# LLNL/ExaConstit

Measured on AMD Instinct MI355X. Metric: quadrature-point constitutive updates/s + Newton-PCG iter/s, 128^3 hex RVE, higher is better.
Workload: dtype f64

## Files before the change

### exaconstit_amd/csrc/capi.hip

```cpp
#include <climits>
#include "exa_internal.hpp"
#include <cstring>
#include <cstdio>

int exa_launch_model_setup(exa_ctx*, double, double*, const double*, const double*, const double*, const double*, double*, double*, double*, hipStream_t);
int exa_launch_model_setup_rec(exa_ctx*, double, double*, const double*, const double*, const double*, const double*, double*, double*, hipStream_t);
int exa_launch_model_setup_p2(exa_ctx*, double, double*, const double*, const double*, const double*, const double*, double*, double*, double*, bool, hipStream_t);
int exa_launch_model_setup_aos_rec(exa_ctx*, double, double*, const double*, const double*, const double*, const double*, double*, double*, hipStream_t);
int exa_launch_init_state(exa_ctx*, double*, const double*, const double*, hipStream_t);
int exa_launch_state_normalize(exa_ctx*, double*, hipStream_t);
int exa_launch_nfev_hist(exa_ctx*, const double*, int*, hipStream_t);
int exa_launch_selftest_km_math(const double*, double*, int, hipStream_t);
int exa_launch_calc_dp(exa_ctx*, const double*, double*, hipStream_t);
int exa_launch_jacobians(exa_ctx*, const double*, double*, hipStream_t);
int exa_launch_jacobians_from_geom(exa_ctx*, const double*, double*, hipStream_t);
int exa_launch_grad_calc(exa_ctx*, const double*, const double*, double*, hipStream_t);
int exa_launch_residual_setup(exa_ctx*, const double*, const double*, hipStream_t);
int exa_launch_residual_apply(exa_ctx*, double*, hipStream_t);
int exa_launch_residual_p1(exa_ctx*, const double*, const double*, double*, bool, hipStream_t);
int exa_launch_grad_setup_pa(exa_ctx*, double, const double*, const double*, hipStream_t);
int exa_launch_grad_apply_p1(exa_ctx*, const double*, double*, bool, const uint8_t*, const double*, hipStream_t, bool trans = false, int blk0 = 0, int nblk_range = -1);
int exa_launch_grad_diag_p1(exa_ctx*, double*, hipStream_t);
int exa_launch_assemble_ea_p1(exa_ctx*, hipStream_t);
int exa_launch_ea_apply_p1(exa_ctx*, const double*, double*, bool, const uint8_t*, const double*, hipStream_t);
int exa_launch_ea_diag_p1(exa_ctx*, double*, hipStream_t);
int exa_launch_ea_export_p1(exa_ctx*, double*, hipStream_t);
int exa_launch_restrict(exa_ctx*, const double*, double*, hipStream_t);
// ... 37 lines not shown
      if (!told) { told = true; std::fprintf(stderr, "exaconstit_hip: Kocks-Mecking kinetics with p = %g, q = %g: the regime p, q != 1 is not pinned to a reference vector (DESIGN.md section 5)\n", ctx->mp.p, ctx->mp.q); }
   }
   exa_build_ref_elem(ctx->p, ctx->G_host, ctx->W_host);
   bool ok = true;
   ok = ok && hipMalloc(&ctx->G_dev, sizeof(double) * ctx->G_host.size()) == hipSuccess;
   ok = ok && hipMalloc(&ctx->W_dev, sizeof(double) * ctx->W_host.size()) == hipSuccess;
   ok = ok && hipMalloc(&ctx->fail_count_dev, sizeof(int)) == hipSuccess;
   ctx->scratch_bytes = sizeof(double) * VOL_AVG_BLOCKS * 64;
   ok = ok && hipMalloc(&ctx->scratch_dev, ctx->scratch_bytes) == hipSuccess;
   if (ok) {
      ok = ok && hipMemcpy(ctx->G_dev, ctx->G_host.data(), sizeof(double) * ctx->G_host.size(), hipMemcpyHostToDevice) == hipSuccess;
      ok = ok && hipMemcpy(ctx->W_dev, ctx->W_host.data(), sizeof(double) * ctx->W_host.size(), hipMemcpyHostToDevice) == hipSuccess;
      ok = ok && hipMemset(ctx->fail_count_dev, 0, sizeof(int)) == hipSuccess;
   }
   if (!ok) { std::fprintf(stderr, "exa_create: device allocation failed\n"); exa_destroy(ctx); set(EXA_ERR_HIP); return nullptr; }
   set(EXA_OK);
   return ctx;
}

void exa_destroy(exa_ctx* ctx) {
   if (!ctx) return;
   (void)hipFree(ctx->n2e_off); (void)hipFree(ctx->n2e_idx); (void)hipFree(ctx->ev_det);
   (void)hipFree(ctx->G_dev); (void)hipFree(ctx->W_dev); (void)hipFree(ctx->fail_count_dev); (void)hipFree(ctx->tail_dev); (void)hipFree(ctx->tail2_dev); (void)hipFree(ctx->resume_dev[0]); (void)hipFree(ctx->resume_dev[1]); (void)hipFree(ctx->scratch_dev);
   (void)hipFree(ctx->dmat); (void)hipFree(ctx->pa); (void)hipFree(ctx->emat); (void)hipFree(ctx->eDS); (void)hipFree(ctx->T1_dev); (void)hipFree(ctx->pa_c); (void)hipFree(ctx->tbuf); (void)hipFree(ctx->vgrad_ref);
   delete ctx;
}

const char* exa_last_error(const exa_ctx* ctx) { return ctx ? ctx->err.c_str() : "null context"; }
int exa_num_state_vars(const exa_ctx* ctx) { return ctx ? ctx->nstatev : EXA_ERR_ARG; }
int exa_nodes_per_elem(const exa_ctx* ctx) { return ctx ? ctx->n : EXA_ERR_ARG; }
int exa_qpts_per_elem(const exa_ctx* ctx) { return ctx ? ctx->Q : EXA_ERR_ARG; }

int exa_shape_table(const exa_ctx* ctx, double* G_host, double* W_host) {
   if (!ctx) return EXA_ERR_ARG;
   if (G_host) std::memcpy(G_host, ctx->G_host.data(), sizeof(double) * ctx->G_host.size());
   if (W_host) std::memcpy(W_host, ctx->W_host.data(), sizeof(double) * ctx->W_host.size());
   return EXA_OK;
}

int exa_set_quadrature_layout(exa_ctx* ctx, int layout) {
   if (!ctx || (layout != EXA_QLAYOUT_AOS && layout != EXA_QLAYOUT_EB64)) return fail(ctx, EXA_ERR_ARG, "exa_set_quadrature_layout: bad argument");
   if (layout == EXA_QLAYOUT_EB64 && !((ctx->p == 1 && ctx->cfg.integ == EXA_INTEG_FULL) || ctx->p == 2))
      return fail(ctx, EXA_ERR_UNSUPPORTED, "exa_set_quadrature_layout: the element-blocked layout is built for p = 1 full integration and for p = 2");
   ctx->qblk = (layout == EXA_QLAYOUT_EB64); ctx->have_resid = false; ctx->have_grad = false;
   return EXA_OK;
}
// ... 16 lines not shown

extern "C" int exa_choose_newton_cap(const int* hist64, double tail_cost);
static int cap_controller(exa_ctx* ctx, int rc, const double* state1, exa_stream s) {
   if (rc != EXA_OK || !ctx->cap_auto) return rc;
   ctx->cap_calls++;
   if (!(ctx->cap_calls <= 4 || ctx->cap_calls % 4 == 0)) return rc;
   int h[64];
   if (int r = exa_model_nfev_hist(ctx, state1, h, s)) return r;
   return exa_set_newton_caps(ctx, exa_choose_newton_cap(h, ctx->cap_tail_cost), 0, ctx->tail_resume);
}

int exa_set_newton_cap_auto(exa_ctx* ctx, int mode, double tail_cost) {
   if (!ctx || mode < 0 || mode > 2) return fail(ctx, EXA_ERR_ARG, "exa_set_newton_cap_auto: mode 0 (off), 1 (Kocks-Mecking models only) or 2 (every model)");
   if (mode && ctx->P >= (int64_t)INT32_MAX) return fail(ctx, EXA_ERR_ARG, "exa_set_newton_cap_auto: the deferred-point list holds 32-bit point ids (P < 2^31)");
   const bool km = ecmdev::kin_is_km(ctx->mp.kin);
   ctx->cap_auto = (mode == 2 || (mode == 1 && km)) ? 1 : 0;
   ctx->cap_tail_cost = tail_cost > 0.0 ? tail_cost : (km ? 1.5 : 4.0);
   ctx->cap_calls = 0;
   if (!mode) { ctx->newton_cap = 0; ctx->newton_cap2 = 0; }
   return EXA_OK;
}
int exa_get_newton_cap(exa_ctx* ctx) { return ctx ? ctx->newton_cap : EXA_ERR_ARG; }

int exa_model_setup(exa_ctx* ctx, double dt, const double* J, const double* vel, const double* stress0, const double* state0,
                    double* stress1, double* state1, double* ddsdde, exa_stream s) {
   if (!ctx || !J || !vel || !stress0 || !state0 || !stress1 || !state1 || !ddsdde) return fail(ctx, EXA_ERR_ARG, "exa_model_setup: null pointer");
   if (!(dt > 0.0)) return fail(ctx, EXA_ERR_ARG, "exa_model_setup: dt must be positive");
   return cap_controller(ctx, exa_launch_model_setup(ctx, dt, const_cast<double*>(J), vel, nullptr, stress0, state0, stress1, state1, ddsdde, S(s)), state1, s);
}

int exa_model_setup_lvec(exa_ctx* ctx, double dt, const double* x_lvec, const double* v_lvec, const double* stress0, const double* state0,
                         double* stress1, double* state1, double* ddsdde, double* J_out, exa_stream s) {
   if (!ctx || !x_lvec || !v_lvec || !stress0 || !state0 || !stress1 || !state1 || !ddsdde || !J_out) return fail(ctx, EXA_ERR_ARG, "exa_model_setup_lvec: null pointer");
   if (!ctx->conn) return fail(ctx, EXA_ERR_STATE, "exa_model_setup_lvec: call exa_set_connectivity first");
   if (!(dt > 0.0)) return fail(ctx, EXA_ERR_ARG, "exa_model_setup_lvec: dt must be positive");
   return cap_controller(ctx, exa_launch_model_setup(ctx, dt, J_out, v_lvec, x_lvec, stress0, state0, stress1, state1, ddsdde, S(s)), state1, s);
}

int exa_model_setup_lvec_records(exa_ctx* ctx, double dt, const double* x_lvec, const double* v_lvec, const double* stress0, const double* state0,
                                 double* stress1, double* state1, double* J_out, exa_stream s) {
   if (!ctx || !x_lvec || !v_lvec || !stress0 || !state0 || !stress1 || !state1) return fail(ctx, EXA_ERR_ARG, "exa_model_setup_lvec_records: null pointer");
   if (!ctx->conn) return fail(ctx, EXA_ERR_STATE, "exa_model_setup_lvec_records: call exa_set_connectivity first");
   if (!(dt > 0.0)) return fail(ctx, EXA_ERR_ARG, "exa_model_setup_lvec_records: dt must be positive");
   const bool p1 = ctx->p == 1 && ctx->cfg.integ == EXA_INTEG_FULL, p2 = ctx->p == 2;
   if (!(p1 || p2) || (!ctx->qblk && !p1) || ctx->tangent_form != EXA_TANGENT_DEV5_BULK || !(ctx->cfg.assembly == EXA_ASSEMBLY_PA || ctx->ea_matfree))
      return fail(ctx, EXA_ERR_UNSUPPORTED, "exa_model_setup_lvec_records: needs p = 1 full integration (either layout) or p = 2 (element-blocked layout), the compact tangent form and PA or matrix-free EA");
   if (p2 && !J_out) return fail(ctx, EXA_ERR_ARG, "exa_model_setup_lvec_records: at p = 2 the Jacobian field is not optional (the pre-pass writes it, the launch and the residual read it)");
   const int npair = p1 ? PAC_PAIRS : PAC_PAIRS_GEO;
   if (ctx->pa_c && ctx->pac_pairs != npair) return fail(ctx, EXA_ERR_STATE, "exa_model_setup_lvec_records: compact records of another shape exist");
   if (!ctx->pa_c) {
      ctx->pac_pairs = npair;
      EXA_HIP_CHECK(ctx, hipMalloc(&ctx->pa_c, (size_t)((ctx->E + PA_BLK - 1) / PA_BLK) * ctx->Q * 2 * npair * PA_BLK * sizeof(double)));
      EXA_HIP_CHECK(ctx, hipMemsetAsync(ctx->pa_c, 0, (size_t)((ctx->E + PA_BLK - 1) / PA_BLK) * ctx->Q * 2 * npair * PA_BLK * sizeof(double), S(s)));
   }
   const int rc = p2 ? exa_launch_model_setup_p2(ctx, dt, J_out, v_lvec, x_lvec, stress0, state0, stress1, state1, nullptr, true, S(s))
                     : !ctx->qblk ? exa_launch_model_setup_aos_rec(ctx, dt, J_out, v_lvec, x_lvec, stress0, state0, stress1, state1, S(s))
                     : exa_launch_model_setup_rec(ctx, dt, J_out, v_lvec, x_lvec, stress0, state0, stress1, state1, S(s));
   if (rc == EXA_OK) { ctx->have_grad = true; ctx->emat_valid = false; ctx->grad_records_only = true; }
   return cap_controller(ctx, rc, state1, s);
}

const int* exa_model_fail_counter_dev(exa_ctx* ctx) { return ctx ? ctx->fail_count_dev : nullptr; }

int exa_model_status(exa_ctx* ctx, exa_stream s) {
   if (!ctx) return EXA_ERR_ARG;
   int h = 0;
// ... 27 lines not shown
   EXA_HIP_CHECK(ctx, hipStreamSynchronize(S(s)));
   return EXA_OK;
}
int exa_selftest_km_math(const double* x_dev, double* out_dev, int n, exa_stream s) {
   if (!x_dev || !out_dev || n <= 0) return EXA_ERR_ARG;
   return exa_launch_selftest_km_math(x_dev, out_dev, n, S(s));
}
int exa_model_tail_count(exa_ctx* ctx, exa_stream s) {
   if (!ctx) return EXA_ERR_ARG;
   if (!ctx->tail_dev || ctx->newton_cap <= 0) return 0;
   int h = 0;
   EXA_HIP_CHECK(ctx, hipMemcpyAsync(&h, ctx->tail_dev, sizeof(int), hipMemcpyDeviceToHost, S(s)));
   EXA_HIP_CHECK(ctx, hipStreamSynchronize(S(s)));
   return h;
}

int exa_calc_dp(exa_ctx* ctx, const double* state, double* dp, exa_stream s) {
   if (!ctx || !state || !dp) return fail(ctx, EXA_ERR_ARG, "exa_calc_dp: null pointer");
   return exa_launch_calc_dp(ctx, state, dp, S(s));
}

int exa_jacobians(exa_ctx* ctx, const double* xe, double* J, exa_stream s) {
   if (!ctx || !xe || !J) return fail(ctx, EXA_ERR_ARG, "exa_jacobians: null pointer");
   return exa_launch_jacobians(ctx, xe, J, S(s));
}

int exa_jacobians_from_geom(exa_ctx* ctx, const double* gj, double* J, exa_stream s) {
   if (!ctx || !gj || !J) return fail(ctx, EXA_ERR_ARG, "exa_jacobians_from_geom: null pointer");
   return exa_launch_jacobians_from_geom(ctx, gj, J, S(s));
}

int exa_grad_calc(exa_ctx* ctx, const double* J, const double* fe, double* out, exa_stream s) {
   if (!ctx || !J || !fe || !out) return fail(ctx, EXA_ERR_ARG, "exa_grad_calc: null pointer");
   return exa_launch_grad_calc(ctx, J, fe, out, S(s));
}

int exa_residual_setup(exa_ctx* ctx, const double* J, const double* stress1, exa_stream s) {
   if (!ctx || !J || !stress1) return fail(ctx, EXA_ERR_ARG, "exa_residual_setup: null pointer");
   if (ctx->qblk) return fail(ctx, EXA_ERR_UNSUPPORTED, "exa_residual_setup: E-vector residual is AOS-only; with the element-blocked layout use exa_residual_lvec");
   ctx->have_resid = true;
   if (ctx->cfg.integ == EXA_INTEG_BBAR) {
      if (!ctx->eDS) EXA_HIP_CHECK(ctx, hipMalloc(&ctx->eDS, sizeof(double) * 3 * ctx->n * PA_BLK * (size_t)((ctx->E + PA_BLK - 1) / PA_BLK)));
      ctx->resid_J = J; ctx->resid_S = stress1;
      return exa_launch_eds(ctx, J, S(s));
   }
   if (!ctx->dmat) EXA_HIP_CHECK(ctx, hipMalloc(&ctx->dmat, sizeof(double) * 9 * ctx->P));
   return exa_launch_residual_setup(ctx, J, stress1, S(s));
}

int exa_residual_apply(exa_ctx* ctx, double* y, exa_stream s) {
   if (!ctx || !y) return fail(ctx, EXA_ERR_ARG, "exa_residual_apply: null pointer");
// ... 43 lines not shown

int exa_set_ea_matrix_free(exa_ctx* ctx, int on) {
   if (!ctx) return EXA_ERR_ARG;
   ctx->ea_matfree = on != 0; return EXA_OK;
}

int exa_grad_setup(exa_ctx* ctx, double dt, const double* J, const double* C, exa_stream s) {
   if (!ctx || !J || !C) return fail(ctx, EXA_ERR_ARG, "exa_grad_setup: null pointer");
   if (!ctx->pa) { EXA_HIP_CHECK(ctx, hipMalloc(&ctx->pa, pa_bytes(ctx->E, ctx->Q))); EXA_HIP_CHECK(ctx, hipMemsetAsync(ctx->pa, 0, pa_bytes(ctx->E, ctx->Q), S(s))); }
   if (ctx->tangent_form == EXA_TANGENT_DEV5_BULK_GEO && !ctx->pa_c) {
      ctx->pac_pairs = PAC_PAIRS_GEO;
      EXA_HIP_CHECK(ctx, hipMalloc(&ctx->pa_c, (size_t)((ctx->E + PA_BLK - 1) / PA_BLK) * ctx->Q * 2 * ctx->pac_pairs * PA_BLK * sizeof(double)));
   }
   if (ctx->tangent_form == EXA_TANGENT_DEV5_BULK && !ctx->pa_c) {
      const bool p1 = ctx->p == 1 && ctx->cfg.integ == EXA_INTEG_FULL && (ctx->cfg.assembly == EXA_ASSEMBLY_PA || ctx->ea_matfree);
      const bool p2 = ctx->n == 27 && (ctx->cfg.assembly == EXA_ASSEMBLY_PA || ctx->ea_matfree);
      if (p1 || p2) {
         ctx->pac_pairs = p1 ? PAC_PAIRS : PAC_PAIRS_GEO;
         EXA_HIP_CHECK(ctx, hipMalloc(&ctx->pa_c, (size_t)((ctx->E + PA_BLK - 1) / PA_BLK) * ctx->Q * 2 * ctx->pac_pairs * PA_BLK * sizeof(double)));
      }
   }
   int rc = exa_launch_grad_setup_pa(ctx, dt, J, C, S(s));
   if (rc) return rc;
   ctx->grad_records_only = false;
   if (ctx->cfg.assembly == EXA_ASSEMBLY_EA) {
      const bool bbar = ctx->cfg.integ == EXA_INTEG_BBAR;
      ctx->ea_generic = bbar || ctx->p != 1;
      if (bbar) {
         if (!ctx->eDS) EXA_HIP_CHECK(ctx, hipMalloc(&ctx->eDS, sizeof(double) * 3 * ctx->n * PA_BLK * (size_t)((ctx->E + PA_BLK - 1) / PA_BLK)));
         rc = exa_launch_eds(ctx, J, S(s));
         if (rc) return rc;
      }
      ctx->emat_valid = false;
      if (!ea_from_records(ctx)) rc = assemble_ea(ctx, S(s));
   } else if (ctx->p != 1) {
      if (!ctx->tbuf) EXA_HIP_CHECK(ctx, hipMalloc(&ctx->tbuf, sizeof(double) * 9 * ctx->P));
   }
   ctx->have_grad = (rc == EXA_OK);
   return rc;
}

int exa_grad_apply(exa_ctx* ctx, const double* x, double* y, exa_stream s) {
   if (!ctx || !x || !y) return fail(ctx, EXA_ERR_ARG, "exa_grad_apply: null pointer");
   if (!ctx->have_grad) return fail(ctx, EXA_ERR_STATE, "exa_grad_apply called before exa_grad_setup");
   if (ctx->grad_records_only) return fail(ctx, EXA_ERR_STATE, "exa_grad_apply: the gradient data are the compact records of exa_model_setup_lvec_records; call exa_grad_setup for the full records");
   if (ctx->cfg.assembly == EXA_ASSEMBLY_EA) {
// ... 136 lines not shown
```

### exaconstit_amd/csrc/exa_internal.hpp

```cpp
#pragma once
#include <hip/hip_runtime.h>
#include <string>
#include <vector>
#include <cstdint>
#include <cstdlib>
#include "../../include/exaconstit_hip.h"
#include "ecm_device.hpp"

#define EXA_HIP_CHECK(ctx, call)                                                                 \
   do {                                                                                          \
      hipError_t e_ = (call);                                                                    \
      if (e_ != hipSuccess) { (ctx)->err = std::string(#call) + ": " + hipGetErrorString(e_); return EXA_ERR_HIP; } \
   } while (0)

constexpr int PA_SLOTS = 46;
constexpr int PA_PAIRS = 23;
constexpr int PA_BLK = 64;

struct exa_ctx {
   exa_config cfg;
   ecmdev::MatParams mp;
   int p, n, Q, E;
   int64_t P;
   int nstatev;
   int device;
   std::string err;
   std::vector<double> G_host, W_host;
   double* G_dev = nullptr; double* W_dev = nullptr;
   double* dmat = nullptr;
   double* pa = nullptr;
   double* emat = nullptr;
   double* T1_dev = nullptr;
   double* eDS = nullptr;
   double* tbuf = nullptr;
   double* vgrad_ref = nullptr;
   const double* resid_J = nullptr; const double* resid_S = nullptr;
   bool ea_generic = false;
   bool ea_matfree = false, emat_valid = false;
   bool qblk = false;
   bool aos_stage = true;
   bool have_resid = false, have_grad = false;
   bool pa_lazy = false; const double* lazy_J = nullptr; const double* lazy_C = nullptr; double lazy_dt = 0.0;
   bool grad_records_only = false;
   const int32_t* conn = nullptr; int nnodes = 0;
   double* pa_c = nullptr;
   int tangent_form = 0;
   int pac_pairs = 0;
   int det = 0; int32_t* n2e_off = nullptr; int32_t* n2e_idx = nullptr; double* ev_det = nullptr; int det_nnodes = 0; const int32_t* det_conn = nullptr;
   const double* coords_lvec = nullptr;
   int* fail_count_dev = nullptr;
   int newton_cap = 0; int* tail_dev = nullptr;
   int newton_cap2 = 0; int* tail2_dev = nullptr;
   int tail_resume = 1; double* resume_dev[2] = { nullptr, nullptr };
   int cap_auto = 0; double cap_tail_cost = 0.0; long cap_calls = 0;
   double* scratch_dev = nullptr; size_t scratch_bytes = 0;
   double hist_init[ecmdev::NUM_HIST];
};

int exa_ensure_p2_tables(struct exa_ctx* ctx);
void exa_build_ref_elem(int p, std::vector<double>& G, std::vector<double>& W);
void exa_build_1d_tables(int p, std::vector<double>& T1, std::vector<int>& nat);
bool exa_fill_mat_params(const exa_config& cfg, ecmdev::MatParams& mp, double* hist_init, std::string& err);

struct QView { int64_t base; int stride; };
template <bool QB>
// ... 84 lines not shown
```

### exaconstit_amd/csrc/pa_kernels.hip

```cpp
#include "exa_internal.hpp"
#include <cstdlib>
#include <cstring>

namespace {

constexpr double GL0 = 0.21132486540518713, GL1 = 0.78867513459481287;
constexpr double gl_pt(int i) { return i == 0 ? GL0 : GL1; }
constexpr int VX[8] = { 0, 1, 1, 0, 0, 1, 1, 0 }, VY[8] = { 0, 0, 1, 1, 0, 0, 1, 1 }, VZ[8] = { 0, 0, 0, 0, 1, 1, 1, 1 };
constexpr double n1(int v, double x) { return v ? x : 1.0 - x; }
constexpr double d1(int v) { return v ? 1.0 : -1.0; }
constexpr double G1(int a, int j, int q) {
   const double x = gl_pt(q & 1), y = gl_pt((q >> 1) & 1), z = gl_pt((q >> 2) & 1);
   return j == 0 ? d1(VX[a]) * n1(VY[a], y) * n1(VZ[a], z) : (j == 1 ? n1(VX[a], x) * d1(VY[a]) * n1(VZ[a], z) : n1(VX[a], x) * n1(VY[a], y) * d1(VZ[a]));
}

__device__ __forceinline__ int64_t pa_off(int64_t blk, int Q, int q, int pair) { return (((blk * Q + q) * PA_PAIRS + pair) * PA_BLK) * 2; }

__device__ __forceinline__ void adj_det(const double* Jq, double adj[9], double& detJ, const int st = 1) {
   const double J11 = Jq[0], J21 = Jq[st], J31 = Jq[2 * st], J12 = Jq[3 * st], J22 = Jq[4 * st], J32 = Jq[5 * st], J13 = Jq[6 * st], J23 = Jq[7 * st], J33 = Jq[8 * st];
   adj[0] = J22 * J33 - J23 * J32; adj[1] = J32 * J13 - J12 * J33; adj[2] = J12 * J23 - J22 * J13;
   adj[3] = J31 * J23 - J21 * J33; adj[4] = J11 * J33 - J13 * J31; adj[5] = J21 * J13 - J11 * J23;
   adj[6] = J21 * J32 - J31 * J22; adj[7] = J31 * J12 - J11 * J32; adj[8] = J11 * J22 - J12 * J21;
   detJ = J11 * adj[0] + J21 * adj[1] + J31 * adj[2];
}
// ... 95 lines not shown
      if (FULL) {
      double2* rec = reinterpret_cast<double2*>(pa + pa_off(blk, Q, q, 0)) + lane;
#pragma unroll
      for (int pr = 0; pr < 18; pr++) rec[pr * PA_BLK] = make_double2(c[(2 * pr) * vc.stride] * sc, c[(2 * pr + 1) * vc.stride] * sc);
#pragma unroll
      for (int pr = 0; pr < 4; pr++) rec[(18 + pr) * PA_BLK] = make_double2(adj[2 * pr], adj[2 * pr + 1]);
      rec[22 * PA_BLK] = make_double2(adj[8], W[q] * detJ);
      }
      if (CMP) {
         double D[36], Dn[25]; tangent_to_d55(c, vc.stride, Dn, D[25]);
#pragma unroll
         for (int l = 0; l < 5; l++)
#pragma unroll
            for (int k = 0; k < 5; k++) D[k + 5 * l] = (TRD ? Dn[l + 5 * k] : Dn[k + 5 * l]) * sc;
         D[25] *= sc;
         if (CMP == PAC_PAIRS_GEO) { for (int i = 0; i < 9; i++) D[26 + i] = adj[i]; D[35] = W[q] * detJ; }
         double2* rc = reinterpret_cast<double2*>(pac + pac_off<CMP ? CMP : 1>(blk, Q, q, 0)) + lane;
#pragma unroll
         for (int pr = 0; pr < CMP; pr++) rc[pr * PA_BLK] = make_double2(D[2 * pr], D[2 * pr + 1]);
      }
   }
}

template <bool QB>
__global__ void k_tangent_defect(const int Q, const int64_t P, const double* __restrict__ C, unsigned long long* __restrict__ out) {
   const int64_t ip = (int64_t)blockIdx.x * blockDim.x + threadIdx.x;
   double defect = 0.0;
   if (ip < P) {
      const QView vc = qview<QB>(36, Q, ip / Q, (int)(ip % Q));
      const double* c = C + vc.base;
      double D[25], K; tangent_to_d55(c, vc.stride, D, K);
      double cmax = 0.0, dmax = 0.0;
#pragma unroll
      for (int j = 0; j < 6; j++) {
         double eps[6] = { 0, 0, 0, 0, 0, 0 }, col[6]; eps[j] = 1.0;
         d55_apply(D, K, eps, col);
#pragma unroll
         for (int i = 0; i < 6; i++) { const double v = c[(i + 6 * j) * vc.stride]; cmax = fmax(cmax, fabs(v)); dmax = fmax(dmax, fabs(v - col[i])); }
      }
      defect = cmax > 0.0 ? dmax / cmax : 0.0;
   }
   for (int o = 32; o > 0; o >>= 1) defect = fmax(defect, __shfl_xor(defect, o));
   if ((threadIdx.x & 63) == 0 && defect > 0.0) atomicMax(out, (unsigned long long)__double_as_longlong(defect));
}

template <bool LVEC, bool GEO, bool CMP = false, bool TRANS = false, bool NT = true, bool CG = false>
// ... 352 lines not shown
                                  const double* __restrict__ qf, double* __restrict__ partial) {
   extern __shared__ double sm[];
   const int nb = gridDim.x;
   for (int c = 0; c <= vdim; c++) {
      double acc = 0;
      for (int64_t ip = (int64_t)blockIdx.x * blockDim.x + threadIdx.x; ip < P; ip += (int64_t)nb * blockDim.x) {
         const int q = (int)(ip % Q); const int64_t e = ip / Q;
         const QView vj = qview<QB>(9, Q, e, q), vq = qview<QB>(vdim, Q, e, q);
         double adj[9], detJ; adj_det(J + vj.base, adj, detJ, vj.stride);
         const double w = W[q] * detJ;
         acc += (c < vdim) ? w * qf[vq.base + (int64_t)c * vq.stride] : w;
      }
      sm[threadIdx.x] = acc; __syncthreads();
      for (int s = blockDim.x / 2; s > 0; s >>= 1) { if ((int)threadIdx.x < s) sm[threadIdx.x] += sm[threadIdx.x + s]; __syncthreads(); }
      if (threadIdx.x == 0) partial[c * nb + blockIdx.x] = sm[0];
      __syncthreads();
   }
}

}

static inline unsigned nblk(int64_t n, int bs) { return (unsigned)((n + bs - 1) / bs); }

int exa_launch_jacobians(exa_ctx* ctx, const double* xe, double* J, hipStream_t s) {
   if (ctx->qblk) hipLaunchKernelGGL(k_jacobians<true>, dim3(nblk(ctx->P, 256)), dim3(256), exa_g_lds_bytes(ctx->n, ctx->Q), s, ctx->Q, ctx->n, ctx->P, ctx->G_dev, xe, J);
   else hipLaunchKernelGGL(k_jacobians<false>, dim3(nblk(ctx->P, 256)), dim3(256), exa_g_lds_bytes(ctx->n, ctx->Q), s, ctx->Q, ctx->n, ctx->P, ctx->G_dev, xe, J);
   EXA_HIP_CHECK(ctx, hipGetLastError()); return EXA_OK;
}
int exa_launch_jacobians_from_geom(exa_ctx* ctx, const double* gj, double* J, hipStream_t s) {
   if (ctx->qblk) hipLaunchKernelGGL(k_jacobians_from_geom<true>, dim3(nblk(ctx->P, 256)), dim3(256), 0, s, ctx->Q, ctx->P, gj, J);
   else hipLaunchKernelGGL(k_jacobians_from_geom<false>, dim3(nblk(ctx->P, 256)), dim3(256), 0, s, ctx->Q, ctx->P, gj, J);
   EXA_HIP_CHECK(ctx, hipGetLastError()); return EXA_OK;
}
int exa_launch_grad_calc(exa_ctx* ctx, const double* J, const double* fe, double* out, hipStream_t s) {
   if (ctx->qblk) hipLaunchKernelGGL(k_grad_calc<true>, dim3(nblk(ctx->P, 256)), dim3(256), exa_g_lds_bytes(ctx->n, ctx->Q), s, ctx->Q, ctx->n, ctx->P, J, ctx->G_dev, fe, out);
   else hipLaunchKernelGGL(k_grad_calc<false>, dim3(nblk(ctx->P, 256)), dim3(256), exa_g_lds_bytes(ctx->n, ctx->Q), s, ctx->Q, ctx->n, ctx->P, J, ctx->G_dev, fe, out);
   EXA_HIP_CHECK(ctx, hipGetLastError()); return EXA_OK;
}
int exa_launch_residual_setup(exa_ctx* ctx, const double* J, const double* S, hipStream_t s) {
   hipLaunchKernelGGL(k_residual_setup, dim3(nblk(ctx->P, 256)), dim3(256), 0, s, ctx->Q, ctx->P, ctx->W_dev, J, S, ctx->dmat);
   EXA_HIP_CHECK(ctx, hipGetLastError()); return EXA_OK;
}
int exa_launch_residual_apply(exa_ctx* ctx, double* Y, hipStream_t s) {
   hipLaunchKernelGGL(k_residual_apply, dim3(nblk((int64_t)ctx->n * ctx->E, 256)), dim3(256), exa_g_lds_bytes(ctx->n, ctx->Q), s, ctx->Q, ctx->n, ctx->E, ctx->G_dev, ctx->dmat, Y);
   EXA_HIP_CHECK(ctx, hipGetLastError()); return EXA_OK;
}
// ... 1 lines not shown
   hipLaunchKernelGGL(k_residual_apply, dim3(nblk((int64_t)ctx->n * ctx->E, 256)), dim3(256), exa_g_lds_bytes(ctx->n, ctx->Q), s, ctx->Q, ctx->n, ctx->E, ctx->G_dev, D, Y);
   EXA_HIP_CHECK(ctx, hipGetLastError()); return EXA_OK;
}
int exa_det_prepare(exa_ctx* ctx);
static int det_gather(exa_ctx* ctx, double* y, const double* gate, hipStream_t s) {
   hipLaunchKernelGGL(k_e2l_gather<true>, dim3(nblk(ctx->nnodes, 256)), dim3(256), 0, s, ctx->n, ctx->nnodes, ctx->n2e_off, ctx->n2e_idx, ctx->ev_det, y, gate);
   EXA_HIP_CHECK(ctx, hipGetLastError()); return EXA_OK;
}
int exa_launch_residual_p1(exa_ctx* ctx, const double* J, const double* S, double* y, bool lvec, hipStream_t s) {
   const unsigned nb = nblk(ctx->E, PA_BLK);
   double* ev = nullptr;
   if (lvec && ctx->det) { if (int rc = exa_det_prepare(ctx)) return rc; ev = ctx->ev_det; }
   if (lvec && J == nullptr) {
      if (ctx->qblk) hipLaunchKernelGGL((k_residual_p1<true, true, true>), dim3(nb), dim3(PA_BLK), 0, s, ctx->E, ctx->W_dev, J, S, y, ctx->conn, ctx->nnodes, ev, ctx->coords_lvec);
      else hipLaunchKernelGGL((k_residual_p1<true, false, true>), dim3(nb), dim3(PA_BLK), 0, s, ctx->E, ctx->W_dev, J, S, y, ctx->conn, ctx->nnodes, ev, ctx->coords_lvec);
   } else if (lvec && ctx->qblk) hipLaunchKernelGGL((k_residual_p1<true, true>), dim3(nb), dim3(PA_BLK), 0, s, ctx->E, ctx->W_dev, J, S, y, ctx->conn, ctx->nnodes, ev);
   else if (lvec) hipLaunchKernelGGL((k_residual_p1<true, false>), dim3(nb), dim3(PA_BLK), 0, s, ctx->E, ctx->W_dev, J, S, y, ctx->conn, ctx->nnodes, ev);
   else if (ctx->qblk) hipLaunchKernelGGL((k_residual_p1<false, true>), dim3(nb), dim3(PA_BLK), 0, s, ctx->E, ctx->W_dev, J, S, y, ctx->conn, ctx->nnodes);
   else hipLaunchKernelGGL((k_residual_p1<false, false>), dim3(nb), dim3(PA_BLK), 0, s, ctx->E, ctx->W_dev, J, S, y, ctx->conn, ctx->nnodes);
   EXA_HIP_CHECK(ctx, hipGetLastError());
   if (ev) return det_gather(ctx, y, nullptr, s);
   return EXA_OK;
}
static int pa_full_on_demand(exa_ctx* ctx, hipStream_t s) {
   if (!ctx->pa_lazy) return EXA_OK;
   const dim3 grid(nblk(ctx->E, PA_BLK));
   if (ctx->qblk) hipLaunchKernelGGL((k_grad_setup_pa<true, 0, false>), grid, dim3(PA_BLK), 0, s, ctx->Q, ctx->E, ctx->lazy_dt, ctx->W_dev, ctx->lazy_J, ctx->lazy_C, ctx->pa, ctx->pa_c);
   else hipLaunchKernelGGL((k_grad_setup_pa<false, 0, false>), grid, dim3(PA_BLK), 0, s, ctx->Q, ctx->E, ctx->lazy_dt, ctx->W_dev, ctx->lazy_J, ctx->lazy_C, ctx->pa, ctx->pa_c);
   EXA_HIP_CHECK(ctx, hipGetLastError());
   ctx->pa_lazy = false;
   return EXA_OK;
}

int exa_launch_grad_setup_pa(exa_ctx* ctx, double dt, const double* J, const double* C, hipStream_t s) {
   ctx->pa_lazy = false;
   const dim3 grid(nblk(ctx->E, PA_BLK));
#define GS_LAUNCH(QBV, NP, TR) hipLaunchKernelGGL((k_grad_setup_pa<QBV, NP, TR>), grid, dim3(PA_BLK), 0, s, ctx->Q, ctx->E, dt, ctx->W_dev, J, C, ctx->pa, ctx->pa_c)
#define GS_LAUNCH2(NP, TR) do { if (ctx->qblk) GS_LAUNCH(true, NP, TR); else GS_LAUNCH(false, NP, TR); } while (0)
   const bool trd = ctx->cfg.assembly == EXA_ASSEMBLY_EA;
   static const bool lazy_off = [] { const char* e = std::getenv("EXA_GRAD_SETUP_LAZY"); return e && std::strcmp(e, "off") == 0; }();
   if (ctx->pa_c && ctx->pac_pairs == PAC_PAIRS && !trd && !lazy_off) {
      if (ctx->qblk) hipLaunchKernelGGL((k_grad_setup_pa<true, PAC_PAIRS, false, false>), grid, dim3(PA_BLK), 0, s, ctx->Q, ctx->E, dt, ctx->W_dev, J, C, ctx->pa, ctx->pa_c);
      else hipLaunchKernelGGL((k_grad_setup_pa<false, PAC_PAIRS, false, false>), grid, dim3(PA_BLK), 0, s, ctx->Q, ctx->E, dt, ctx->W_dev, J, C, ctx->pa, ctx->pa_c);
      ctx->pa_lazy = true; ctx->lazy_J = J; ctx->lazy_C = C; ctx->lazy_dt = dt;
   }
   else if (ctx->pa_c && ctx->pac_pairs == PAC_PAIRS_GEO && ctx->n == 8 && !trd && !lazy_off) {
      if (ctx->qblk) hipLaunchKernelGGL((k_grad_setup_pa<true, PAC_PAIRS_GEO, false, false>), grid, dim3(PA_BLK), 0, s, ctx->Q, ctx->E, dt, ctx->W_dev, J, C, ctx->pa, ctx->pa_c);
      else hipLaunchKernelGGL((k_grad_setup_pa<false, PAC_PAIRS_GEO, false, false>), grid, dim3(PA_BLK), 0, s, ctx->Q, ctx->E, dt, ctx->W_dev, J, C, ctx->pa, ctx->pa_c);
      ctx->pa_lazy = true; ctx->lazy_J = J; ctx->lazy_C = C; ctx->lazy_dt = dt;
   }
   else if (ctx->pa_c && ctx->pac_pairs == PAC_PAIRS) { if (trd) GS_LAUNCH2(PAC_PAIRS, true); else GS_LAUNCH2(PAC_PAIRS, false); }
   else if (ctx->pa_c) { if (trd) GS_LAUNCH2(PAC_PAIRS_GEO, true); else GS_LAUNCH2(PAC_PAIRS_GEO, false); }
   else GS_LAUNCH2(0, false);
#undef GS_LAUNCH2
#undef GS_LAUNCH
   EXA_HIP_CHECK(ctx, hipGetLastError()); return EXA_OK;
}
int exa_launch_grad_apply_p1(exa_ctx* ctx, const double* x, double* y, bool lvec, const uint8_t* mask, const double* gate, hipStream_t s, bool trans, int blk0, int nblk_range) {
   const unsigned nball = nblk(ctx->E, PA_BLK);
   const bool ranged = nblk_range >= 0;
   if (ranged && (!lvec || ctx->det || blk0 < 0 || (unsigned)(blk0 + nblk_range) > nball)) { ctx->err = "exa_launch_grad_apply_p1: block ranges are for the atomic L-vector action"; return EXA_ERR_ARG; }
   const unsigned nb = ranged ? (unsigned)nblk_range : nball;
   if (!ranged) blk0 = 0;
   if (nb == 0) return EXA_OK;
   if (!(lvec && ctx->coords_lvec && ctx->pa_c && ctx->pac_pairs == PAC_PAIRS) && !(!lvec && ctx->pa_c && ctx->pac_pairs == PAC_PAIRS_GEO && ctx->n == 8)) {
      if (int rc = pa_full_on_demand(ctx, s)) return rc;
   }
   double* ev = nullptr;
   if (lvec && ctx->det) { if (int rc = exa_det_prepare(ctx)) return rc; ev = ctx->ev_det; }
   const bool nt = exa_stream_nt((size_t)ctx->P * 16 * ((lvec && ctx->coords_lvec && ctx->pa_c && ctx->pac_pairs == PAC_PAIRS) ? PAC_PAIRS : ((lvec && ctx->coords_lvec) ? 18 : PA_PAIRS)));
#define GA_LAUNCH(G, CM, T, REC, CRD) do { if (nt) hipLaunchKernelGGL((k_grad_apply_p1<true, G, CM, T, true>), dim3(nb), dim3(PA_BLK), 0, s, ctx->E, REC, x, y, ctx->conn, ctx->nnodes, mask, gate, CRD, ev, blk0); \
      else hipLaunchKernelGGL((k_grad_apply_p1<true, G, CM, T, false>), dim3(nb), dim3(PA_BLK), 0, s, ctx->E, REC, x, y, ctx->conn, ctx->nnodes, mask, gate, CRD, ev, blk0); } while (0)
   const double* none = nullptr;
   if (lvec && ctx->coords_lvec && ctx->pa_c && ctx->pac_pairs == PAC_PAIRS) GA_LAUNCH(true, true, false, ctx->pa_c, ctx->coords_lvec);
   else if (lvec && ctx->coords_lvec) { if (trans) GA_LAUNCH(true, false, true, ctx->pa, ctx->coords_lvec); else GA_LAUNCH(true, false, false, ctx->pa, ctx->coords_lvec); }
   else if (lvec) { if (trans) GA_LAUNCH(false, false, true, ctx->pa, none); else GA_LAUNCH(false, false, false, ctx->pa, none); }
   else if (ctx->pa_c && ctx->pac_pairs == PAC_PAIRS_GEO && ctx->n == 8)
// ... 17 lines not shown
}
int exa_launch_assemble_ea_p1(exa_ctx* ctx, hipStream_t s) {
   hipLaunchKernelGGL(k_assemble_ea_p1, dim3(nblk(ctx->E, PA_BLK), 24), dim3(PA_BLK), 0, s, ctx->E, ctx->pa, ctx->emat);
   EXA_HIP_CHECK(ctx, hipGetLastError()); return EXA_OK;
}
int exa_launch_ea_apply_p1(exa_ctx* ctx, const double* x, double* y, bool lvec, const uint8_t* mask, const double* gate, hipStream_t s) {
   const unsigned nb = nblk(ctx->E, PA_BLK);
   if (lvec) hipLaunchKernelGGL(k_ea_apply_p1<true>, dim3(nb), dim3(PA_BLK), 0, s, ctx->E, ctx->emat, x, y, ctx->conn, ctx->nnodes, mask, gate);
   else hipLaunchKernelGGL(k_ea_apply_p1<false>, dim3(nb), dim3(PA_BLK), 0, s, ctx->E, ctx->emat, x, y, ctx->conn, ctx->nnodes, mask, gate);
   EXA_HIP_CHECK(ctx, hipGetLastError()); return EXA_OK;
}
int exa_launch_ea_diag_p1(exa_ctx* ctx, double* y, hipStream_t s) {
   hipLaunchKernelGGL(k_ea_diag_p1, dim3(nblk(ctx->E, PA_BLK)), dim3(PA_BLK), 0, s, ctx->E, ctx->emat, y);
   EXA_HIP_CHECK(ctx, hipGetLastError()); return EXA_OK;
}
int exa_launch_ea_export_p1(exa_ctx* ctx, double* out, hipStream_t s) {
   hipLaunchKernelGGL(k_ea_export_p1, dim3(nblk(ctx->E, PA_BLK)), dim3(PA_BLK), 0, s, ctx->E, ctx->emat, out);
   EXA_HIP_CHECK(ctx, hipGetLastError()); return EXA_OK;
}
int exa_launch_restrict(exa_ctx* ctx, const double* L, double* Ev, hipStream_t s) {
   hipLaunchKernelGGL(k_restrict, dim3(nblk((int64_t)ctx->n * ctx->E, 256)), dim3(256), 0, s, ctx->n, ctx->E, ctx->nnodes, ctx->conn, L, Ev);
   EXA_HIP_CHECK(ctx, hipGetLastError()); return EXA_OK;
}
int exa_launch_restrict_T(exa_ctx* ctx, const double* Ev, double* L, hipStream_t s) {
   if (ctx->det) {
      if (int rc = exa_det_prepare(ctx)) return rc;
      hipLaunchKernelGGL(k_e2l_gather<false>, dim3(nblk(ctx->nnodes, 256)), dim3(256), 0, s, ctx->n, ctx->nnodes, ctx->n2e_off, ctx->n2e_idx, Ev, L, (const double*)nullptr);
      EXA_HIP_CHECK(ctx, hipGetLastError()); return EXA_OK;
   }
   hipLaunchKernelGGL(k_restrict_T, dim3(nblk((int64_t)ctx->n * ctx->E, 256)), dim3(256), 0, s, ctx->n, ctx->E, ctx->nnodes, ctx->conn, Ev, L);
   EXA_HIP_CHECK(ctx, hipGetLastError()); return EXA_OK;
}
int exa_launch_vol_avg(exa_ctx* ctx, const double* J, const double* qf, int vdim, double* partial, int nb, hipStream_t s) {
   if (ctx->qblk) hipLaunchKernelGGL(k_vol_avg_partial<true>, dim3(nb), dim3(256), sizeof(double) * 256, s, ctx->Q, ctx->P, vdim, ctx->W_dev, J, qf, partial);
   else hipLaunchKernelGGL(k_vol_avg_partial<false>, dim3(nb), dim3(256), sizeof(double) * 256, s, ctx->Q, ctx->P, vdim, ctx->W_dev, J, qf, partial);
   EXA_HIP_CHECK(ctx, hipGetLastError()); return EXA_OK;
}
```

Measured before the change: 3.883 billion.

## Stage grad-setup inputs through LDS and use gather-based E-to-L transpose by default

Adds a grad-setup kernel that loads per-point J and C rows through shared memory with coalesced double2 loads before building PA/compact records, used for the point-major Q=8 layout. The element-to-L-vector transpose now defaults to the node-ordered gather (n2e CSR) instead of atomic scatter, preparing the map during grad setup. It also makes the lazy full-PA build safe across streams with an event, and guards model/jacobian outputs that alias the lazily referenced J/C buffers. This trades extra LDS use and a one-time CSR build for less uncoalesced traffic and fewer atomics, with added sync logic risk.

```diff
diff --git a/exaconstit_amd/csrc/capi.hip b/exaconstit_amd/csrc/capi.hip
--- a/exaconstit_amd/csrc/capi.hip
+++ b/exaconstit_amd/csrc/capi.hip
@@ -1,8 +1,12 @@
 #include <climits>
+#include <initializer_list>
+#include <utility>
 #include "exa_internal.hpp"
 #include <cstring>
 #include <cstdio>
 
+int exa_pa_full_on_demand(exa_ctx* ctx, hipStream_t s);
+int exa_e2l_prepare(exa_ctx* ctx, hipStream_t s);
 int exa_launch_model_setup(exa_ctx*, double, double*, const double*, const double*, const double*, const double*, double*, double*, double*, hipStream_t);
 int exa_launch_model_setup_rec(exa_ctx*, double, double*, const double*, const double*, const double*, const double*, double*, double*, hipStream_t);
 int exa_launch_model_setup_p2(exa_ctx*, double, double*, const double*, const double*, const double*, const double*, double*, double*, double*, bool, hipStream_t);
@@ -86,6 +90,7 @@
    if (!ctx) return;
    (void)hipFree(ctx->n2e_off); (void)hipFree(ctx->n2e_idx); (void)hipFree(ctx->ev_det);
    (void)hipFree(ctx->G_dev); (void)hipFree(ctx->W_dev); (void)hipFree(ctx->fail_count_dev); (void)hipFree(ctx->tail_dev); (void)hipFree(ctx->tail2_dev); (void)hipFree(ctx->resume_dev[0]); (void)hipFree(ctx->resume_dev[1]); (void)hipFree(ctx->scratch_dev);
+   if (ctx->lazy_ev) (void)hipEventDestroy(ctx->lazy_ev);
    (void)hipFree(ctx->dmat); (void)hipFree(ctx->pa); (void)hipFree(ctx->emat); (void)hipFree(ctx->eDS); (void)hipFree(ctx->T1_dev); (void)hipFree(ctx->pa_c); (void)hipFree(ctx->tbuf); (void)hipFree(ctx->vgrad_ref);
    delete ctx;
 }
@@ -148,10 +153,22 @@
 }
 int exa_get_newton_cap(exa_ctx* ctx) { return ctx ? ctx->newton_cap : EXA_ERR_ARG; }
 
+static int lazy_guard(exa_ctx* ctx, std::initializer_list<std::pair<const double*, int64_t>> outs, hipStream_t s) {
+   if (!ctx->pa_lazy) return EXA_OK;
+   auto hits = [](const double* a, int64_t na, const double* b, int64_t nb) { return a && b && a < b + nb && b < a + na; };
+   for (const auto& o : outs)
+      if (hits(o.first, o.second, ctx->lazy_J, 9 * ctx->P) || hits(o.first, o.second, ctx->lazy_C, 36 * ctx->P)) return exa_pa_full_on_demand(ctx, s);
+   return EXA_OK;
+}
+static int lazy_guard_model(exa_ctx* ctx, const double* J_out, double* stress1, double* state1, double* ddsdde, hipStream_t s) {
+   return lazy_guard(ctx, { { J_out, 9 * ctx->P }, { stress1, 6 * ctx->P }, { state1, (int64_t)ctx->nstatev * ctx->P }, { ddsdde, 36 * ctx->P } }, s);
+}
+
 int exa_model_setup(exa_ctx* ctx, double dt, const double* J, const double* vel, const double* stress0, const double* state0,
                     double* stress1, double* state1, double* ddsdde, exa_stream s) {
    if (!ctx || !J || !vel || !stress0 || !state0 || !stress1 || !state1 || !ddsdde) return fail(ctx, EXA_ERR_ARG, "exa_model_setup: null pointer");
    if (!(dt > 0.0)) return fail(ctx, EXA_ERR_ARG, "exa_model_setup: dt must be positive");
+   if (int rc = lazy_guard_model(ctx, nullptr, stress1, state1, ddsdde, S(s))) return rc;
    return cap_controller(ctx, exa_launch_model_setup(ctx, dt, const_cast<double*>(J), vel, nullptr, stress0, state0, stress1, state1, ddsdde, S(s)), state1, s);
 }
 
@@ -160,6 +177,7 @@
    if (!ctx || !x_lvec || !v_lvec || !stress0 || !state0 || !stress1 || !state1 || !ddsdde || !J_out) return fail(ctx, EXA_ERR_ARG, "exa_model_setup_lvec: null pointer");
    if (!ctx->conn) return fail(ctx, EXA_ERR_STATE, "exa_model_setup_lvec: call exa_set_connectivity first");
    if (!(dt > 0.0)) return fail(ctx, EXA_ERR_ARG, "exa_model_setup_lvec: dt must be positive");
+   if (int rc = lazy_guard_model(ctx, J_out, stress1, state1, ddsdde, S(s))) return rc;
    return cap_controller(ctx, exa_launch_model_setup(ctx, dt, J_out, v_lvec, x_lvec, stress0, state0, stress1, state1, ddsdde, S(s)), state1, s);
 }
 
@@ -168,6 +186,7 @@
    if (!ctx || !x_lvec || !v_lvec || !stress0 || !state0 || !stress1 || !state1) return fail(ctx, EXA_ERR_ARG, "exa_model_setup_lvec_records: null pointer");
    if (!ctx->conn) return fail(ctx, EXA_ERR_STATE, "exa_model_setup_lvec_records: call exa_set_connectivity first");
    if (!(dt > 0.0)) return fail(ctx, EXA_ERR_ARG, "exa_model_setup_lvec_records: dt must be positive");
+   if (int rc = lazy_guard_model(ctx, J_out, stress1, state1, nullptr, S(s))) return rc;
    const bool p1 = ctx->p == 1 && ctx->cfg.integ == EXA_INTEG_FULL, p2 = ctx->p == 2;
    if (!(p1 || p2) || (!ctx->qblk && !p1) || ctx->tangent_form != EXA_TANGENT_DEV5_BULK || !(ctx->cfg.assembly == EXA_ASSEMBLY_PA || ctx->ea_matfree))
       return fail(ctx, EXA_ERR_UNSUPPORTED, "exa_model_setup_lvec_records: needs p = 1 full integration (either layout) or p = 2 (element-blocked layout), the compact tangent form and PA or matrix-free EA");
@@ -241,11 +260,13 @@
 
 int exa_jacobians(exa_ctx* ctx, const double* xe, double* J, exa_stream s) {
    if (!ctx || !xe || !J) return fail(ctx, EXA_ERR_ARG, "exa_jacobians: null pointer");
+   if (int rc = lazy_guard(ctx, { { J, 9 * ctx->P } }, S(s))) return rc;
    return exa_launch_jacobians(ctx, xe, J, S(s));
 }
 
 int exa_jacobians_from_geom(exa_ctx* ctx, const double* gj, double* J, exa_stream s) {
    if (!ctx || !gj || !J) return fail(ctx, EXA_ERR_ARG, "exa_jacobians_from_geom: null pointer");
+   if (int rc = lazy_guard(ctx, { { J, 9 * ctx->P } }, S(s))) return rc;
    return exa_launch_jacobians_from_geom(ctx, gj, J, S(s));
 }
 
@@ -335,6 +356,7 @@
    }
    int rc = exa_launch_grad_setup_pa(ctx, dt, J, C, S(s));
    if (rc) return rc;
+   if (ctx->conn && (rc = exa_e2l_prepare(ctx, S(s)))) return rc;
    ctx->grad_records_only = false;
    if (ctx->cfg.assembly == EXA_ASSEMBLY_EA) {
       const bool bbar = ctx->cfg.integ == EXA_INTEG_BBAR;
diff --git a/exaconstit_amd/csrc/exa_internal.hpp b/exaconstit_amd/csrc/exa_internal.hpp
--- a/exaconstit_amd/csrc/exa_internal.hpp
+++ b/exaconstit_amd/csrc/exa_internal.hpp
@@ -41,6 +41,7 @@
    bool aos_stage = true;
    bool have_resid = false, have_grad = false;
    bool pa_lazy = false; const double* lazy_J = nullptr; const double* lazy_C = nullptr; double lazy_dt = 0.0;
+   hipStream_t lazy_stream = nullptr; hipEvent_t lazy_ev = nullptr;
    bool grad_records_only = false;
    const int32_t* conn = nullptr; int nnodes = 0;
    double* pa_c = nullptr;
diff --git a/exaconstit_amd/csrc/pa_kernels.hip b/exaconstit_amd/csrc/pa_kernels.hip
--- a/exaconstit_amd/csrc/pa_kernels.hip
+++ b/exaconstit_amd/csrc/pa_kernels.hip
@@ -141,6 +141,71 @@
    }
 }
 
+static bool evec_staged(const char* which) {
+   const char* e = std::getenv("EXA_EVEC_STAGED");
+   if (!e || std::strncmp(e, "off", 3) != 0) return true;
+   return e[3] == ':' && std::strstr(e + 4, which) == nullptr;
+}
+
+template <int NU, int W, int RS, bool NT = true>
+__device__ __forceinline__ void stage_rows_in(double* lds, const double* __restrict__ g, const int n, const int lane) {
+   double2 r[NU];
+#pragma unroll
+   for (int m = 0; m < NU; m++) {
+      const int u = 2 * (m * 64 + lane);
+      r[m] = make_double2(0.0, 0.0);
+      if (u + 1 < n) r[m] = ld_rec<NT>(reinterpret_cast<const double2*>(g + u));
+      else if (u < n) r[m].x = g[u];
+   }
+#pragma unroll
+   for (int m = 0; m < NU; m++) {
+      const int u = 2 * (m * 64 + lane);
+      if (u < n) { const int i0 = (u / W) * RS + u % W; lds[i0] = r[m].x; lds[i0 + 1] = r[m].y; }
+   }
+}
+constexpr int GS_RS_C = 37;
+template <int CMP, bool TRD, bool FULL>
+__global__ __launch_bounds__(PA_BLK) void k_grad_setup_pa_stg(const int E, const double dt, const double* __restrict__ W, const double* __restrict__ J,
+                                                              const double* __restrict__ C, double* __restrict__ pa, double* __restrict__ pac) {
+   constexpr int Q = 8;
+   __shared__ double stg[PA_BLK * GS_RS_C];
+   const int lane = threadIdx.x;
+   const int64_t p0 = (int64_t)blockIdx.x * PA_BLK, P = (int64_t)E * Q;
+   const int nv = (int)(P - p0 < PA_BLK ? P - p0 : PA_BLK);
+   const int64_t e = p0 / Q + (lane >> 3); const int q = lane & 7;
+   const int64_t blk = e / PA_BLK; const int el = (int)(e % PA_BLK);
+   stage_rows_in<5, 18, 18>(stg, J + p0 * 9, nv * 9, lane);
+   __syncthreads();
+   double adj[9], detJ;
+   if (lane < nv) adj_det(stg + 9 * lane, adj, detJ);
+   __syncthreads();
+   stage_rows_in<18, 36, GS_RS_C>(stg, C + p0 * 36, nv * 36, lane);
+   __syncthreads();
+   if (lane >= nv) return;
+   const double sc = dt * W[q] / detJ;
+   const double* c = stg + GS_RS_C * lane;
+   if (FULL) {
+      double2* rec = reinterpret_cast<double2*>(pa + pa_off(blk, Q, q, 0)) + el;
+#pragma unroll
+      for (int pr = 0; pr < 18; pr++) rec[pr * PA_BLK] = make_double2(c[2 * pr] * sc, c[2 * pr + 1] * sc);
+#pragma unroll
+      for (int pr = 0; pr < 4; pr++) rec[(18 + pr) * PA_BLK] = make_double2(adj[2 * pr], adj[2 * pr + 1]);
+      rec[22 * PA_BLK] = make_double2(adj[8], W[q] * detJ);
+   }
+   if (CMP) {
+      double D[36], Dn[25]; tangent_to_d55(c, 1, Dn, D[25]);
+#pragma unroll
+      for (int l = 0; l < 5; l++)
+#pragma unroll
+         for (int k = 0; k < 5; k++) D[k + 5 * l] = (TRD ? Dn[l + 5 * k] : Dn[k + 5 * l]) * sc;
+      D[25] *= sc;
+      if (CMP == PAC_PAIRS_GEO) { for (int i = 0; i < 9; i++) D[26 + i] = adj[i]; D[35] = W[q] * detJ; }
+      double2* rc = reinterpret_cast<double2*>(pac + pac_off<CMP ? CMP : 1>(blk, Q, q, 0)) + el;
+#pragma unroll
+      for (int pr = 0; pr < CMP; pr++) rc[pr * PA_BLK] = make_double2(D[2 * pr], D[2 * pr + 1]);
+   }
+}
+
 template <bool QB>
 __global__ void k_tangent_defect(const int Q, const int64_t P, const double* __restrict__ C, unsigned long long* __restrict__ out) {
    const int64_t ip = (int64_t)blockIdx.x * blockDim.x + threadIdx.x;
@@ -539,6 +604,7 @@
 
 static inline unsigned nblk(int64_t n, int bs) { return (unsigned)((n + bs - 1) / bs); }
 
+static bool al16(const void* p) { return ((uintptr_t)p & 15) == 0; }
 int exa_launch_jacobians(exa_ctx* ctx, const double* xe, double* J, hipStream_t s) {
    if (ctx->qblk) hipLaunchKernelGGL(k_jacobians<true>, dim3(nblk(ctx->P, 256)), dim3(256), exa_g_lds_bytes(ctx->n, ctx->Q), s, ctx->Q, ctx->n, ctx->P, ctx->G_dev, xe, J);
    else hipLaunchKernelGGL(k_jacobians<false>, dim3(nblk(ctx->P, 256)), dim3(256), exa_g_lds_bytes(ctx->n, ctx->Q), s, ctx->Q, ctx->n, ctx->P, ctx->G_dev, xe, J);
@@ -586,37 +652,59 @@
    if (ev) return det_gather(ctx, y, nullptr, s);
    return EXA_OK;
 }
+static bool gs_staged(const exa_ctx* ctx, const double* J, const double* C) { return !ctx->qblk && ctx->Q == 8 && al16(J) && al16(C) && evec_staged("setup"); }
 static int pa_full_on_demand(exa_ctx* ctx, hipStream_t s) {
    if (!ctx->pa_lazy) return EXA_OK;
    const dim3 grid(nblk(ctx->E, PA_BLK));
-   if (ctx->qblk) hipLaunchKernelGGL((k_grad_setup_pa<true, 0, false>), grid, dim3(PA_BLK), 0, s, ctx->Q, ctx->E, ctx->lazy_dt, ctx->W_dev, ctx->lazy_J, ctx->lazy_C, ctx->pa, ctx->pa_c);
+   if (ctx->lazy_stream != s && ctx->lazy_ev) {
+      hipStreamCaptureStatus cs = hipStreamCaptureStatusNone;
+      EXA_HIP_CHECK(ctx, hipStreamIsCapturing(s, &cs));
+      if (cs == hipStreamCaptureStatusNone) EXA_HIP_CHECK(ctx, hipStreamWaitEvent(s, ctx->lazy_ev, 0));
+   }
+   if (gs_staged(ctx, ctx->lazy_J, ctx->lazy_C)) hipLaunchKernelGGL((k_grad_setup_pa_stg<0, false, true>), dim3(nblk(ctx->P, PA_BLK)), dim3(PA_BLK), 0, s, ctx->E, ctx->lazy_dt, ctx->W_dev, ctx->lazy_J, ctx->lazy_C, ctx->pa, ctx->pa_c);
+   else if (ctx->qblk) hipLaunchKernelGGL((k_grad_setup_pa<true, 0, false>), grid, dim3(PA_BLK), 0, s, ctx->Q, ctx->E, ctx->lazy_dt, ctx->W_dev, ctx->lazy_J, ctx->lazy_C, ctx->pa, ctx->pa_c);
    else hipLaunchKernelGGL((k_grad_setup_pa<false, 0, false>), grid, dim3(PA_BLK), 0, s, ctx->Q, ctx->E, ctx->lazy_dt, ctx->W_dev, ctx->lazy_J, ctx->lazy_C, ctx->pa, ctx->pa_c);
    EXA_HIP_CHECK(ctx, hipGetLastError());
    ctx->pa_lazy = false;
    return EXA_OK;
 }
 
+int exa_pa_full_on_demand(exa_ctx* ctx, hipStream_t s) { return pa_full_on_demand(ctx, s); }
+static int lazy_mark(exa_ctx* ctx, double dt, const double* J, const double* C, hipStream_t s) {
+   if (!ctx->lazy_ev) EXA_HIP_CHECK(ctx, hipEventCreateWithFlags(&ctx->lazy_ev, hipEventDisableTiming));
+   hipStreamCaptureStatus cs = hipStreamCaptureStatusNone;
+   EXA_HIP_CHECK(ctx, hipStreamIsCapturing(s, &cs));
+   if (cs == hipStreamCaptureStatusNone) EXA_HIP_CHECK(ctx, hipEventRecord(ctx->lazy_ev, s));
+   ctx->pa_lazy = true; ctx->lazy_J = J; ctx->lazy_C = C; ctx->lazy_dt = dt; ctx->lazy_stream = s;
+   return EXA_OK;
+}
 int exa_launch_grad_setup_pa(exa_ctx* ctx, double dt, const double* J, const double* C, hipStream_t s) {
    ctx->pa_lazy = false;
    const dim3 grid(nblk(ctx->E, PA_BLK));
+   const bool stg = gs_staged(ctx, J, C);
+   const dim3 grid_stg(nblk(ctx->P, PA_BLK));
 #define GS_LAUNCH(QBV, NP, TR) hipLaunchKernelGGL((k_grad_setup_pa<QBV, NP, TR>), grid, dim3(PA_BLK), 0, s, ctx->Q, ctx->E, dt, ctx->W_dev, J, C, ctx->pa, ctx->pa_c)
-#define GS_LAUNCH2(NP, TR) do { if (ctx->qblk) GS_LAUNCH(true, NP, TR); else GS_LAUNCH(false, NP, TR); } while (0)
+#define GS_LAUNCH_STG(NP, TR, FL) hipLaunchKernelGGL((k_grad_setup_pa_stg<NP, TR, FL>), grid_stg, dim3(PA_BLK), 0, s, ctx->E, dt, ctx->W_dev, J, C, ctx->pa, ctx->pa_c)
+#define GS_LAUNCH2(NP, TR) do { if (ctx->qblk) GS_LAUNCH(true, NP, TR); else if (stg) GS_LAUNCH_STG(NP, TR, true); else GS_LAUNCH(false, NP, TR); } while (0)
    const bool trd = ctx->cfg.assembly == EXA_ASSEMBLY_EA;
    static const bool lazy_off = [] { const char* e = std::getenv("EXA_GRAD_SETUP_LAZY"); return e && std::strcmp(e, "off") == 0; }();
    if (ctx->pa_c && ctx->pac_pairs == PAC_PAIRS && !trd && !lazy_off) {
       if (ctx->qblk) hipLaunchKernelGGL((k_grad_setup_pa<true, PAC_PAIRS, false, false>), grid, dim3(PA_BLK), 0, s, ctx->Q, ctx->E, dt, ctx->W_dev, J, C, ctx->pa, ctx->pa_c);
+      else if (stg) GS_LAUNCH_STG(PAC_PAIRS, false, false);
       else hipLaunchKernelGGL((k_grad_setup_pa<false, PAC_PAIRS, false, false>), grid, dim3(PA_BLK), 0, s, ctx->Q, ctx->E, dt, ctx->W_dev, J, C, ctx->pa, ctx->pa_c);
-      ctx->pa_lazy = true; ctx->lazy_J = J; ctx->lazy_C = C; ctx->lazy_dt = dt;
+      if (int rc = lazy_mark(ctx, dt, J, C, s)) return rc;
    }
    else if (ctx->pa_c && ctx->pac_pairs == PAC_PAIRS_GEO && ctx->n == 8 && !trd && !lazy_off) {
       if (ctx->qblk) hipLaunchKernelGGL((k_grad_setup_pa<true, PAC_PAIRS_GEO, false, false>), grid, dim3(PA_BLK), 0, s, ctx->Q, ctx->E, dt, ctx->W_dev, J, C, ctx->pa, ctx->pa_c);
+      else if (stg) GS_LAUNCH_STG(PAC_PAIRS_GEO, false, false);
       else hipLaunchKernelGGL((k_grad_setup_pa<false, PAC_PAIRS_GEO, false, false>), grid, dim3(PA_BLK), 0, s, ctx->Q, ctx->E, dt, ctx->W_dev, J, C, ctx->pa, ctx->pa_c);
-      ctx->pa_lazy = true; ctx->lazy_J = J; ctx->lazy_C = C; ctx->lazy_dt = dt;
+      if (int rc = lazy_mark(ctx, dt, J, C, s)) return rc;
    }
    else if (ctx->pa_c && ctx->pac_pairs == PAC_PAIRS) { if (trd) GS_LAUNCH2(PAC_PAIRS, true); else GS_LAUNCH2(PAC_PAIRS, false); }
    else if (ctx->pa_c) { if (trd) GS_LAUNCH2(PAC_PAIRS_GEO, true); else GS_LAUNCH2(PAC_PAIRS_GEO, false); }
    else GS_LAUNCH2(0, false);
 #undef GS_LAUNCH2
+#undef GS_LAUNCH_STG
 #undef GS_LAUNCH
    EXA_HIP_CHECK(ctx, hipGetLastError()); return EXA_OK;
 }
@@ -680,8 +768,22 @@
    hipLaunchKernelGGL(k_restrict, dim3(nblk((int64_t)ctx->n * ctx->E, 256)), dim3(256), 0, s, ctx->n, ctx->E, ctx->nnodes, ctx->conn, L, Ev);
    EXA_HIP_CHECK(ctx, hipGetLastError()); return EXA_OK;
 }
+static bool e2l_ordered(exa_ctx* ctx, hipStream_t s, int& rc) {
+   rc = EXA_OK;
+   if (ctx->det) return true;
+   if (!evec_staged("transpose") || !ctx->conn) return false;
+   if (ctx->n2e_off && ctx->det_conn == ctx->conn && ctx->det_nnodes == ctx->nnodes) return true;
+   hipStreamCaptureStatus cs = hipStreamCaptureStatusNone;
+   if (hipStreamIsCapturing(s, &cs) != hipSuccess || cs != hipStreamCaptureStatusNone) return false;
+   rc = exa_det_prepare(ctx);
+   return rc == EXA_OK;
+}
+int exa_e2l_prepare(exa_ctx* ctx, hipStream_t s) { int rc; (void)e2l_ordered(ctx, s, rc); return rc; }
 int exa_launch_restrict_T(exa_ctx* ctx, const double* Ev, double* L, hipStream_t s) {
-   if (ctx->det) {
+   int rc;
+   const bool ordered = e2l_ordered(ctx, s, rc);
+   if (rc) return rc;
+   if (ordered) {
       if (int rc = exa_det_prepare(ctx)) return rc;
       hipLaunchKernelGGL(k_e2l_gather<false>, dim3(nblk(ctx->nnodes, 256)), dim3(256), 0, s, ctx->n, ctx->nnodes, ctx->n2e_off, ctx->n2e_idx, Ev, L, (const double*)nullptr);
       EXA_HIP_CHECK(ctx, hipGetLastError()); return EXA_OK;
```

Result: no change. 3.887 billion (median of 6 runs) (+0.1%).
